# jspenmar/slowtv_monodepth

Hardware: AMD Instinct MI355X
Metric: training images/sec (640×192, 3-frame) at 1/2/4/8 MI355X; warp+SSIM HBM GB/s (higher is better)
Workload: dtype f32

## Files before the change

### include/smd_hotpath.h

```cpp
#ifndef SMD_HOTPATH_H
#define SMD_HOTPATH_H

#include <stddef.h>
#include <stdint.h>

#ifdef __cplusplus
extern "C" {
#endif

#define SMD_ABI_VERSION 8

#define SMD_OK 0
#define SMD_E_INVALID (-1)
#define SMD_E_LAUNCH (-2)
#define SMD_E_WORKSPACE (-3)
#define SMD_E_UNSUPPORTED (-4)

#define SMD_USE_MIN 0x1
#define SMD_USE_AUTOMASK 0x2
#define SMD_LOSS_L1 0x4
#define SMD_NEED_K_GRAD 0x8
#define SMD_USE_EDGES 0x10
#define SMD_LOSS_L2 0x20
#define SMD_MASK_EXPLAINABILITY 0x80
// ... 157 lines not shown
                                int B, int C, int CO, int h, int w, int pieces, void* stream);

size_t smd_conv3x3z_mfma_workspace_bytes(int B, int C, int CO, int h, int w);
int smd_conv3x3z_mfma_fwd(const float* x, const void* wp_fwd, float* y, void* workspace, size_t workspace_bytes,
                          int B, int C, int CO, int h, int w, int pieces, void* stream);
int smd_conv3x3z_mfma_bwd_data(const float* g_y, const void* wp_bwd, float* g_x, void* workspace, size_t workspace_bytes,
                               int B, int C, int CO, int h, int w, int pieces, void* stream);
int smd_conv3x3z_mfma_bwd_weight(const float* x, const float* g_y, float* g_weight, void* workspace, size_t workspace_bytes,
                                 int B, int C, int CO, int h, int w, int pieces, void* stream);

size_t smd_conv7x7s2_packed_bytes(int C, int CO);
size_t smd_conv7x7s2_workspace_bytes(int B, int C, int CO, int H, int W);
int smd_conv7x7s2_pack(const float* weight, void* wp, int C, int CO, void* stream);
int smd_conv7x7s2_fwd(const float* x, const void* wp, float* y, int B, int C, int CO, int H, int W, void* stream);
int smd_conv7x7s2_bwd_weight(const float* x, const float* g_y, float* g_weight, void* workspace, size_t workspace_bytes,
                             int B, int C, int CO, int H, int W, void* stream);

size_t smd_conv3x3s2_mfma_workspace_bytes(int B, int C, int CO, int H, int W);
int smd_conv3x3s2_mfma_fwd(const float* x, const void* wp_fwd, float* y, void* workspace, size_t workspace_bytes,
                           int B, int C, int CO, int H, int W, void* stream);
int smd_conv3x3s2_mfma_bwd_weight(const float* x, const float* g_y, float* g_weight, void* workspace, size_t workspace_bytes,
                                  int B, int C, int CO, int H, int W, void* stream);

size_t smd_bn_workspace_bytes(int N, int C, int HW);
int smd_bn_fwd(const float* x, const float* residual, const float* gamma, const float* beta, float* running_mean, float* running_var,
               float momentum, float eps, int relu, float* y, float* save_mean, float* save_invstd,
               void* workspace, size_t workspace_bytes, int N, int C, int HW, void* stream);
int smd_bn_bwd(const float* x, const float* y, const float* g_y, const float* gamma, const float* save_mean, const float* save_invstd,
               int relu, float* g_x, float* g_residual, float* g_gamma, float* g_beta,
               void* workspace, size_t workspace_bytes, int N, int C, int HW, void* stream);

int smd_maxpool3x3s2_fwd(const float* x, float* y, uint8_t* idx, int N, int C, int H, int W, void* stream);
int smd_maxpool3x3s2_bwd(const float* g_y, const uint8_t* idx, float* g_x, int N, int C, int H, int W, void* stream);

size_t smd_dwconv7x7_workspace_bytes(int C, int H, int W);
int smd_dwconv7x7_fwd(const float* x, const float* weight, const float* bias, float* y, int N, int C, int H, int W, int flip, void* stream);
int smd_dwconv7x7_wrw(const float* x, const float* g_y, float* g_weight, float* g_bias, void* workspace, size_t workspace_bytes,
                      int N, int C, int H, int W, void* stream);

size_t smd_layernorm_cf_workspace_bytes(int N, int C, int HW);
int smd_layernorm_cf_fwd(const float* x, const float* gamma, const float* beta, void* y, int y_is_bf16, float* mean, float* rstd,
                         int N, int C, int HW, float eps, void* stream);
int smd_layernorm_cf_bwd(const float* x, const void* g_y, int g_y_is_bf16, const float* gamma, const float* mean, const float* rstd,
                         float* g_x, float* g_gamma, float* g_beta, void* workspace, size_t workspace_bytes, int N, int C, int HW, void* stream);

size_t smd_channel_attention_workspace_bytes(int B, int C, int n, int backward);
// ... 114 lines not shown
```

### slowtv_monodepth_amd/_lib.py

```python
from __future__ import annotations

import ctypes as C
import os
from pathlib import Path

import torch

__all__ = ['lib', 'call', 'set_knob', 'reset_knobs', 'knob_epoch', 'lib_path', 'FLAGS', 'REGR_FLAGS', 'SEL_MASKED', 'ptr_array', 'int_array', 'i64_array', 'HotpathError', 'Unsupported']

_HERE = Path(__file__).resolve().parent
lib_path = Path(os.environ.get('SMD_HOTPATH_LIB', _HERE/'libsmd_hotpath.so'))

FLAGS = {'use_min': 0x1, 'use_automask': 0x2, 'loss_l1': 0x4, 'need_k_grad': 0x8, 'use_edges': 0x10, 'loss_l2': 0x20, 'packed_ready': 0x40,
         'mask_explainability': 0x80, 'mask_uncertainty': 0x100, 'use_laplacian': 0x200, 'bwd_skip_rows': 0x400, 'edges_ready': 0x800, 'bwd_no_live': 0x1000}
REGR_FLAGS = {'l1': 0x0, 'log_l1': 0x1, 'berhu': 0x2, 'invert': 0x4, 'automask': 0x8}
SEL_MASKED = 255
MAX_SCALES = 8
MAX_SUPPORTS = 8

_vp, _i, _f, _sz, _u64 = C.c_void_p, C.c_int, C.c_float, C.c_size_t, C.c_uint64

PROTOTYPES = {
    'smd_last_error': (C.c_char_p, []),
    'smd_abi_version': (_i, []),
# ... 50 lines not shown
    'smd_scale_mean_fwd': (_i, [_vp]*2 + [_i]*2 + [_vp]*2 + [_sz, _vp]),
    'smd_scale_mean_bwd': (_i, [_vp]*2 + [_i]*2 + [_vp]*3),
    'smd_conv3x3_thin_workspace_bytes': (_sz, [_i]*4),
    'smd_conv3x3_thin_fwd': (_i, [_vp]*3 + [_i]*4 + [_vp]),
    'smd_conv3x3_thin_bwd': (_i, [_vp]*6 + [_sz] + [_i]*4 + [_vp]),
    'smd_conv3x3_mfma_packed_bytes': (_sz, [_i]*3),
    'smd_conv3x3_mfma_workspace_bytes': (_sz, [_i]*5),
    'smd_conv3x3_mfma_pack': (_i, [_vp]*3 + [_i]*3 + [_vp]),
    'smd_conv3x3_mfma_fwd': (_i, [_vp]*4 + [_sz] + [_i]*6 + [_vp]),
    'smd_conv3x3_mfma_bwd_data': (_i, [_vp]*4 + [_sz] + [_i]*6 + [_vp]),
    'smd_conv3x3_mfma_bwd_weight': (_i, [_vp]*4 + [_sz] + [_i]*6 + [_vp]),
    'smd_conv3x3z_mfma_workspace_bytes': (_sz, [_i]*5),
    'smd_conv3x3z_mfma_fwd': (_i, [_vp]*4 + [_sz] + [_i]*6 + [_vp]),
    'smd_conv3x3z_mfma_bwd_data': (_i, [_vp]*4 + [_sz] + [_i]*6 + [_vp]),
    'smd_conv3x3z_mfma_bwd_weight': (_i, [_vp]*4 + [_sz] + [_i]*6 + [_vp]),
    'smd_conv7x7s2_packed_bytes': (_sz, [_i]*2),
    'smd_conv7x7s2_workspace_bytes': (_sz, [_i]*5),
    'smd_conv7x7s2_pack': (_i, [_vp]*2 + [_i]*2 + [_vp]),
    'smd_conv7x7s2_fwd': (_i, [_vp]*3 + [_i]*5 + [_vp]),
    'smd_conv7x7s2_bwd_weight': (_i, [_vp]*4 + [_sz] + [_i]*5 + [_vp]),
    'smd_conv3x3s2_mfma_workspace_bytes': (_sz, [_i]*5),
    'smd_conv3x3s2_mfma_fwd': (_i, [_vp]*4 + [_sz] + [_i]*5 + [_vp]),
    'smd_conv3x3s2_mfma_bwd_weight': (_i, [_vp]*4 + [_sz] + [_i]*5 + [_vp]),
    'smd_conv3x3_head_workspace_bytes': (_sz, [_i]*4),
    'smd_conv3x3_head_fwd': (_i, [_vp]*4 + [_i]*5 + [_vp]),
    'smd_conv3x3_head_bwd': (_i, [_vp]*8 + [_sz] + [_i]*5 + [_vp]),
    'smd_elu_pad_fwd': (_i, [_vp]*3 + [_i]*6 + [_vp]),
    'smd_elu_pad_bwd': (_i, [_vp]*6 + [_sz] + [_i]*6 + [_vp]),
    'smd_elu_up_cat_pad_fwd': (_i, [_vp]*4 + [_i]*6 + [_vp]),
    'smd_elu_up_cat_pad_bwd': (_i, [_vp]*7 + [_sz] + [_i]*6 + [_vp]),
    'smd_bn_workspace_bytes': (_sz, [_i, _i, _i]),
    'smd_bn_fwd': (_i, [_vp]*6 + [_f, _f, _i] + [_vp]*4 + [_sz] + [_i]*3 + [_vp]),
    'smd_bn_bwd': (_i, [_vp]*6 + [_i] + [_vp]*5 + [_sz] + [_i]*3 + [_vp]),
    'smd_maxpool3x3s2_fwd': (_i, [_vp]*3 + [_i]*4 + [_vp]),
    'smd_maxpool3x3s2_bwd': (_i, [_vp]*3 + [_i]*4 + [_vp]),
    'smd_dwconv7x7_workspace_bytes': (_sz, [_i]*3),
    'smd_dwconv7x7_fwd': (_i, [_vp]*4 + [_i]*5 + [_vp]),
    'smd_dwconv7x7_wrw': (_i, [_vp]*5 + [_sz] + [_i]*4 + [_vp]),
    'smd_layernorm_cf_workspace_bytes': (_sz, [_i]*3),
    'smd_layernorm_cf_fwd': (_i, [_vp]*4 + [_i] + [_vp]*2 + [_i]*3 + [_f, _vp]),
    'smd_layernorm_cf_bwd': (_i, [_vp]*2 + [_i] + [_vp]*7 + [_sz] + [_i]*3 + [_vp]),
    'smd_channel_attention_workspace_bytes': (_sz, [_i]*4),
    'smd_channel_attention_fwd': (_i, [_vp]*4 + [_sz] + [_i]*3 + [_vp]),
    'smd_channel_attention_bwd': (_i, [_vp]*5 + [_sz] + [_i]*3 + [_vp]),
    'smd_se_gate_workspace_bytes': (_sz, [_i]*3),
    'smd_se_gate_fwd': (_i, [_vp]*8 + [_sz] + [_i]*3 + [_vp]),
# ... 95 lines not shown
```

### slowtv_monodepth_amd/conv_routing.py

```python
from __future__ import annotations

import torch

from ._lib import Unsupported

_MODE = 'auto'
_ROUTES: dict = {}
_AB_WARMUPS, _AB_ROUNDS, _AB_MARGIN = 2, 5, 0.97
_DECLINED = (Unsupported, ValueError)


def set_conv_route(mode: str = 'auto'):
    global _MODE
    if mode not in ('auto', 'mfma', 'miopen'): raise ValueError(mode)
    _MODE = mode
    _ROUTES.clear()


def conv_routes() -> dict:
    return dict(_ROUTES)


_COARSE_W_MAX, _COARSE_C_MIN = 80, 256
_Z_FWD_WGT = [dict(px_min=1000, ch_max=511), dict(px_min=2400)]
STATIC_RULES = {
    'padded': {'fwd': [dict(thin=True), dict(thin=False, px_min=20000, c_co_max=128*64), dict(thin=False, coarse=True, px_min=1000)],
               'data': [dict(thin=True), dict(thin=False, px_min=5000, c_max=256), dict(thin=False, coarse=True, px_min=1000)],
               'wgt': [dict(thin=False, px_min=20000, co_max=64), dict(thin=False, coarse=True, px_min=2400)]},
    'bf16': {'fwd': [dict(thin=True)], 'data': [dict(thin=True)], 'wgt': [dict(thin=True)]},
    'zpad': {'fwd': _Z_FWD_WGT, 'data': [dict(px_min=1000)], 'wgt': _Z_FWD_WGT},
    'stem': {'fwd': [dict(px_min=20000)], 'wgt': [dict(px_min=20000)]},
}
_FAMILY_OF_SUFFIX = {'': 'padded', 'bf16': 'bf16', 'z': 'zpad', 's': 'stem'}
_BOUNDS = {'px_min': lambda v, B, C, CO, h, w: B*h*w >= v,
           'c_max': lambda v, B, C, CO, h, w: C <= v,
           'co_max': lambda v, B, C, CO, h, w: CO <= v,
           'c_co_max': lambda v, B, C, CO, h, w: C*CO <= v,
           'ch_max': lambda v, B, C, CO, h, w: max(C, CO) <= v,
           'thin': lambda v, B, C, CO, h, w: (CO == 16) == v,
           'coarse': lambda v, B, C, CO, h, w: (w <= _COARSE_W_MAX and C >= _COARSE_C_MIN) == v}


STRIDED_RULES = {
    's2': {'fwd': [dict(px_min=5000)], 'wgt': []},
}


def static_rule(op, B, C, CO, h, w) -> bool:
    kind, _, suffix = op.partition('_')
    clauses = STATIC_RULES[_FAMILY_OF_SUFFIX[suffix]][kind] if suffix in _FAMILY_OF_SUFFIX else STRIDED_RULES[suffix][kind]
    return any(all(_BOUNDS[name](v, B, C, CO, h, w) for name, v in clause.items()) for clause in clauses)


_capturing = torch.cuda.is_current_stream_capturing


def _time_interleaved(run_mfma, run_ref, rounds):
    ev = [[torch.cuda.Event(enable_timing=True) for _ in range(3)] for _ in range(rounds)]
    for e in ev:
        e[0].record(); run_mfma(); e[1].record(); run_ref(); e[2].record()
    torch.cuda.synchronize()
    return [e[0].elapsed_time(e[1])*1e3 for e in ev], [e[1].elapsed_time(e[2])*1e3 for e in ev]


def _conv_route(op, B, C, CO, h, w, run_mfma, run_ref) -> bool:
    if _MODE != 'auto': return _MODE == 'mfma'
    key = (op, B, C, CO, h, w)
    r = _ROUTES.get(key)
    if r is None:
        if _capturing(): return static_rule(op, B, C, CO, h, w)
        for _ in range(_AB_WARMUPS): run_mfma(); run_ref()
        us_m, us_r = _time_interleaved(run_mfma, run_ref, _AB_ROUNDS)
        t_m, t_r = sorted(us_m)[_AB_ROUNDS//2], sorted(us_r)[_AB_ROUNDS//2]
        r = _ROUTES[key] = (t_m < _AB_MARGIN*t_r, t_m, t_r)
# ... 18 lines not shown
```

### slowtv_monodepth_amd/conv_s2.py

```python
from __future__ import annotations

import torch

from . import _lib
from ._device import _check, _on, _stream, _workspace, call
from .conv_ops import _mfma_pack
from .conv_routing import serve


class _Conv3x3s2(torch.autograd.Function):
    @staticmethod
    def forward(ctx, x, weight):
        x = _check('x', x)
        if x.ndim != 4: raise ValueError(f'expected (B,C,H,W), got {tuple(x.shape)}')
        B, C, H, W = x.shape
        if weight.ndim != 4 or tuple(weight.shape[1:]) != (C, 3, 3): raise ValueError(f'weight: expected (CO,{C},3,3), got {tuple(weight.shape)}')
        CO = weight.shape[0]
        weight = _check('weight', weight, (CO, C, 3, 3))
        ho, wo = (H - 1)//2 + 1, (W - 1)//2 + 1
        nws = _lib.lib.smd_conv3x3s2_mfma_workspace_bytes(B, C, CO, H, W)
        y = torch.empty((B, CO, ho, wo), device=x.device, dtype=torch.float32)

        def run_mfma():
            wf = _mfma_pack(weight, C, CO, 3, True, False)[0]
            ws, n = _workspace(x.device, nws, floor=256)
            call('smd_conv3x3s2_mfma_fwd', x.data_ptr(), wf.data_ptr(), y.data_ptr(), ws.data_ptr(), n, B, C, CO, H, W, _stream())
            return y
        y = serve(('fwd_s2', B, C, CO, H, W), run_mfma, lambda: torch.conv2d(x, weight, None, 2, 1), eligible=nws > 0)
        ctx.save_for_backward(x, weight)
        ctx.nws = nws
        return y

    @staticmethod
    def backward(ctx, g_y):
        x, weight = ctx.saved_tensors
        dev = _on(x)
        B, C, H, W = x.shape
        CO = weight.shape[0]
        need_x, need_w = ctx.needs_input_grad
        g_y = _check('grad(y)', g_y, (B, CO, (H - 1)//2 + 1, (W - 1)//2 + 1))
        cb = lambda mask: torch.ops.aten.convolution_backward(g_y, x, weight, None, [2, 2], [1, 1], [1, 1], False, [0, 0], 1, mask)
        g_x = cb([True, False, False])[0] if need_x else None
        g_w = None
        if need_w:
            g_w = torch.empty_like(weight)

            def run_wgt():
                ws, n = _workspace(dev, ctx.nws, floor=256)
                call('smd_conv3x3s2_mfma_bwd_weight', x.data_ptr(), g_y.data_ptr(), g_w.data_ptr(), ws.data_ptr(), n, B, C, CO, H, W, _stream())
                return g_w
            g_w = serve(('wgt_s2', B, C, CO, H, W), run_wgt, lambda: cb([False, True, False])[1], eligible=ctx.nws > 0)
        return g_x, g_w


def conv3x3_s2(x, weight):
    return _Conv3x3s2.apply(x, weight)
```

### slowtv_monodepth_amd/csrc/smd_api.hip

```cpp
#include <limits.h>
#include <math.h>
#include <stdarg.h>
#include <stdio.h>
#include <stdlib.h>
#include <string.h>
#include <algorithm>

#include "smd_kernels.h"
#include "smd_smooth_dev.h"

namespace {

thread_local char g_err[512] = "";

int fail(int code, const char* fmt, ...) {
  va_list ap;
  va_start(ap, fmt);
  vsnprintf(g_err, sizeof(g_err), fmt, ap);
  va_end(ap);
  return code;
}

int check_launch(hipError_t e, const char* what) {
  if (e != hipSuccess) return fail(SMD_E_LAUNCH, "%s: %s", what, hipGetErrorString(e));
// ... 871 lines not shown
  if (!g_y || (!g_xp && !g_weight) || (g_xp && !weight) || (g_weight && (!xp || !workspace))) return fail(SMD_E_INVALID, "null pointer");
  if (C != 16 && C != 32 && C >= 1) return fail(SMD_E_UNSUPPORTED, "the thin convolution serves 16 or 32 input channels, not %d", C);
  if (!thin_sizes_ok(B, C, h, w)) return fail(SMD_E_INVALID, "invalid sizes B=%d C=%d h=%d w=%d", B, C, h, w);
  if (g_weight && workspace_bytes < smd_conv3x3_thin_workspace_bytes(B, C, h, w)) return fail(SMD_E_WORKSPACE, "workspace too small");
  hipStream_t st = (hipStream_t)stream;
  if (g_xp) { if (int rc = check_launch(smd::launch_conv_thin_bwd_data(g_y, weight, g_xp, B, C, h, w, st), "conv3x3_thin_bwd (data)")) return rc; }
  if (g_weight) { if (int rc = check_launch(smd::launch_conv_thin_bwd_wgt(xp, g_y, g_weight, (float*)workspace, B, C, h, w, st), "conv3x3_thin_bwd (weights)")) return rc; }
  return SMD_OK;
}
int smd_conv3x3_thin_fwd(const float* xp, const float* weight, float* y, int B, int C, int h, int w, void* stream) {
  if (!xp || !weight || !y) return fail(SMD_E_INVALID, "null pointer");
  if (C != 16 && C != 32 && C >= 1) return fail(SMD_E_UNSUPPORTED, "the thin convolution serves 16 or 32 input channels, not %d", C);
  if (!thin_sizes_ok(B, C, h, w)) return fail(SMD_E_INVALID, "invalid sizes B=%d C=%d h=%d w=%d", B, C, h, w);
  return check_launch(smd::launch_conv_thin_fwd(xp, weight, y, B, C, h, w, (hipStream_t)stream), "conv3x3_thin_fwd");
}
static bool mfma_sizes_ok(int B, int C, int CO, int h, int w) {
  return B >= 1 && C >= 1 && CO >= 1 && C <= 4096 && CO <= 4096 && h >= 1 && w >= 1 && h < 32768 && w < 32768 && (long long)(h + 2)*(w + 2) < (1ll << 30) &&
         (long long)B*((C + 31)/32)*((CO + 31)/32) < 65536 && (long long)C*(h + 2)*(w + 2) < (1ll << 29) && (long long)CO*h*w < (1ll << 29);
}
using smd::ConvOp;
static bool conv_two_tiles() { return knob("conv_two_tiles", 0) != 0; }
size_t smd_conv3x3_mfma_packed_bytes(int C, int CO, int pieces) {
  if (C < 1 || CO < 1 || pieces < 1 || pieces > 3) return 0;
  return align256(smd::conv_mfma_packed_elems(C, CO, pieces)*2);
}
static size_t mfma_workspace_bytes(bool zpad, int B, int C, int CO, int h, int w, bool two_tiles) {
  if (!mfma_sizes_ok(B, C, CO, h, w)) return 0;
  size_t n = std::max({(size_t)64, smd::conv_mfma_split_elems(ConvOp::Fwd, zpad, B, C, CO, h, w, two_tiles), smd::conv_mfma_split_elems(ConvOp::Data, zpad, B, C, CO, h, w, two_tiles)});
  if (smd::conv_mfma_served(ConvOp::Wgt, zpad, C, CO)) n = std::max(n, smd::conv_mfma_wgrad_partials(zpad, B, C, CO, h, w));
  return align256(n*sizeof(float));
}
size_t smd_conv3x3_mfma_workspace_bytes(int B, int C, int CO, int h, int w) { return mfma_workspace_bytes(false, B, C, CO, h, w, conv_two_tiles()); }
size_t smd_conv3x3z_mfma_workspace_bytes(int B, int C, int CO, int h, int w) { return mfma_workspace_bytes(true, B, C, CO, h, w, conv_two_tiles()); }
static int mfma_unserved(ConvOp op, bool zpad, int C, int CO) {
  const char* name[] = {"forward", "data gradient", "weight gradient"};
  return fail(SMD_E_UNSUPPORTED, "the %s%s does not serve C=%d CO=%d", zpad ? "zero-padded " : "", name[(int)op], C, CO);
}
static int mfma_check(ConvOp op, bool zpad, size_t workspace_bytes, int B, int C, int CO, int h, int w, int pieces, bool two_tiles) {
  if (zpad && pieces != 2 && pieces != 3) return fail(SMD_E_UNSUPPORTED, "the zero-padded forms take float tensors: pieces 2 or 3, not %d", pieces);
  if (pieces < 1 || pieces > 3) return fail(SMD_E_UNSUPPORTED, "pieces must be 1 (bfloat16 tensors), 2 or 3 (float tensors), not %d", pieces);
  if (!mfma_sizes_ok(B, C, CO, h, w)) return fail(SMD_E_INVALID, "invalid sizes B=%d C=%d CO=%d h=%d w=%d", B, C, CO, h, w);
  if (!smd::conv_mfma_served(op, zpad, C, CO)) return mfma_unserved(op, zpad, C, CO);
  if (workspace_bytes < mfma_workspace_bytes(zpad, B, C, CO, h, w, two_tiles)) return fail(SMD_E_WORKSPACE, "workspace too small");
  return SMD_OK;
}
int smd_conv3x3_mfma_pack(const float* weight, void* wp_fwd, void* wp_bwd, int C, int CO, int pieces, void* stream) {
  if (!weight || (!wp_fwd && !wp_bwd)) return fail(SMD_E_INVALID, "null pointer");
  if (pieces < 1 || pieces > 3) return fail(SMD_E_UNSUPPORTED, "pieces must be 1 (bfloat16 tensors), 2 or 3 (float tensors), not %d", pieces);
  if (C < 1 || CO < 1 || C > 4096 || CO > 4096) return fail(SMD_E_INVALID, "invalid sizes C=%d CO=%d", C, CO);
  if (wp_fwd && !smd::conv_mfma_served(ConvOp::Fwd, false, C, CO)) return mfma_unserved(ConvOp::Fwd, false, C, CO);
  if (wp_bwd && !smd::conv_mfma_served(ConvOp::Data, false, C, CO)) return mfma_unserved(ConvOp::Data, false, C, CO);
  return check_launch(smd::launch_conv_mfma_pack(weight, wp_fwd, wp_bwd, C, CO, pieces, (hipStream_t)stream), "conv3x3_mfma_pack");
}
static int mfma_form(ConvOp op, bool zpad, const void* in, const void* wp, void* out, void* workspace, size_t workspace_bytes, int B, int C, int CO, int h, int w, int pieces, void* stream, const char* what) {
  if (!in || !wp || !out || !workspace) return fail(SMD_E_INVALID, "null pointer");
  const bool two_tiles = conv_two_tiles();
  if (int rc = mfma_check(op, zpad, workspace_bytes, B, C, CO, h, w, pieces, two_tiles)) return rc;
  const auto launch = op == ConvOp::Fwd ? smd::launch_conv_mfma_fwd : smd::launch_conv_mfma_bwd_data;
  return check_launch(launch(in, wp, out, (float*)workspace, zpad, B, C, CO, h, w, pieces, two_tiles, (hipStream_t)stream), what);
}
static int mfma_bwd_weight(bool zpad, const void* x, const void* g_y, float* g_weight, void* workspace, size_t workspace_bytes, int B, int C, int CO, int h, int w, int pieces, void* stream) {
  if (!x || !g_y || !g_weight || !workspace) return fail(SMD_E_INVALID, "null pointer");
  if (int rc = mfma_check(ConvOp::Wgt, zpad, workspace_bytes, B, C, CO, h, w, pieces, conv_two_tiles())) return rc;
  return check_launch(smd::launch_conv_mfma_bwd_wgt(x, g_y, g_weight, (float*)workspace, zpad, B, C, CO, h, w, pieces, (hipStream_t)stream), zpad ? "conv3x3z_mfma_bwd_weight" : "conv3x3_mfma_bwd_weight");
}
int smd_conv3x3_mfma_fwd(const void* xp, const void* wp_fwd, void* y, void* workspace, size_t workspace_bytes, int B, int C, int CO, int h, int w, int pieces, void* stream) {
  return mfma_form(ConvOp::Fwd, false, xp, wp_fwd, y, workspace, workspace_bytes, B, C, CO, h, w, pieces, stream, "conv3x3_mfma_fwd");
}
int smd_conv3x3_mfma_bwd_data(const void* g_y, const void* wp_bwd, void* g_xp, void* workspace, size_t workspace_bytes, int B, int C, int CO, int h, int w, int pieces, void* stream) {
  return mfma_form(ConvOp::Data, false, g_y, wp_bwd, g_xp, workspace, workspace_bytes, B, C, CO, h, w, pieces, stream, "conv3x3_mfma_bwd_data");
}
int smd_conv3x3_mfma_bwd_weight(const void* xp, const void* g_y, float* g_weight, void* workspace, size_t workspace_bytes, int B, int C, int CO, int h, int w, int pieces, void* stream) {
  return mfma_bwd_weight(false, xp, g_y, g_weight, workspace, workspace_bytes, B, C, CO, h, w, pieces, stream);
}
// ... 39 lines not shown
  if (B < 1 || B > 65535 || C < 1 || CO < 1 || C > 4096 || CO > 4096 || H < 1 || W < 1) return false;
  const long long ho = (H - 1)/2 + 1, wo = (W - 1)/2 + 1;
  return (long long)C*H*W < (1ll << 29) && (long long)CO*ho*wo < (1ll << 29) && ho <= 65535 && (long long)B*((C + 63)/64)*((CO + 63)/64) < 65536;
}
size_t smd_conv3x3s2_mfma_workspace_bytes(int B, int C, int CO, int H, int W) {
  if (!smd::conv_s2_served(C, CO) || !s2_sizes_ok(B, C, CO, H, W)) return 0;
  return align256(smd::conv_s2_workspace_floats(B, C, CO, H, W)*sizeof(float));
}
static int s2_check(size_t workspace_bytes, int B, int C, int CO, int H, int W) {
  if (!smd::conv_s2_served(C, CO)) return fail(SMD_E_UNSUPPORTED, "the stride-2 kernels serve C %% 16 == 0 with CO %% 32 == 0, not C=%d CO=%d", C, CO);
  if (!s2_sizes_ok(B, C, CO, H, W)) return fail(SMD_E_UNSUPPORTED, "the stride-2 kernels do not serve B=%d C=%d CO=%d H=%d W=%d", B, C, CO, H, W);
  if (workspace_bytes < smd_conv3x3s2_mfma_workspace_bytes(B, C, CO, H, W)) return fail(SMD_E_WORKSPACE, "workspace too small");
  return SMD_OK;
}
int smd_conv3x3s2_mfma_fwd(const float* x, const void* wp_fwd, float* y, void* workspace, size_t workspace_bytes, int B, int C, int CO, int H, int W, void* stream) {
  if (!x || !wp_fwd || !y || !workspace) return fail(SMD_E_INVALID, "null pointer");
  if (int rc = s2_check(workspace_bytes, B, C, CO, H, W)) return rc;
  return check_launch(smd::launch_conv_s2_fwd(x, wp_fwd, y, (float*)workspace, B, C, CO, H, W, (hipStream_t)stream), "conv3x3s2_mfma_fwd");
}
int smd_conv3x3s2_mfma_bwd_weight(const float* x, const float* g_y, float* g_weight, void* workspace, size_t workspace_bytes, int B, int C, int CO, int H, int W, void* stream) {
  if (!x || !g_y || !g_weight || !workspace) return fail(SMD_E_INVALID, "null pointer");
  if (int rc = s2_check(workspace_bytes, B, C, CO, H, W)) return rc;
  return check_launch(smd::launch_conv_s2_bwd_wgt(x, g_y, g_weight, (float*)workspace, B, C, CO, H, W, (hipStream_t)stream), "conv3x3s2_mfma_bwd_weight");
}
int smd_elu_up_cat_pad_fwd(const void* a, const float* bias, const void* skip, void* out, int B, int Ca, int Cs, int h, int w, int dtypes, void* stream) {
  if (!a || !out || (Cs > 0 && !skip)) return fail(SMD_E_INVALID, "null pointer");
  if (B < 1 || Ca < 1 || Cs < 0 || h < 1 || w < 1 || !dec_sizes_ok((long long)B*(Ca + Cs), 2*h, 2*w))
    return fail(SMD_E_INVALID, "invalid sizes B=%d Ca=%d Cs=%d h=%d w=%d", B, Ca, Cs, h, w);
  return check_launch(smd::launch_elu_up_cat_pad_fwd(a, bias, skip, out, B, Ca, Cs, h, w, dtypes, (hipStream_t)stream), "elu_up_cat_pad_fwd");
}
int smd_elu_up_cat_pad_bwd(const void* a, const float* bias, const void* g_out, void* g_a, void* g_skip, float* g_bias,
                           void* workspace, size_t workspace_bytes, int B, int Ca, int Cs, int h, int w, int dtypes, void* stream) {
  if (!a || !g_out || (!g_a && !g_skip) || (g_bias && (!workspace || !g_a))) return fail(SMD_E_INVALID, "null pointer");
  if (B < 1 || Ca < 1 || Cs < 0 || h < 1 || w < 1 || !dec_sizes_ok((long long)B*(Ca + Cs), 2*h, 2*w))
    return fail(SMD_E_INVALID, "invalid sizes B=%d Ca=%d Cs=%d h=%d w=%d", B, Ca, Cs, h, w);
  if (g_bias && workspace_bytes < smd_decoder_glue_workspace_bytes(B, Ca, h, w)) return fail(SMD_E_WORKSPACE, "workspace too small");
  return check_launch(smd::launch_elu_up_cat_pad_bwd(a, bias, g_out, g_a, g_skip, g_bias, (float*)workspace, B, Ca, Cs, h, w, dtypes, (hipStream_t)stream),
                      "elu_up_cat_pad_bwd");
}

size_t smd_bn_workspace_bytes(int N, int C, int HW) {
  if (N < 1 || C < 1 || HW < 1) return 0;
  return align256(((size_t)C*smd::bn_chunks(N, HW)*3 + (size_t)C*3)*sizeof(float));
}
int smd_bn_fwd(const float* x, const float* residual, const float* gamma, const float* beta, float* running_mean, float* running_var,
               float momentum, float eps, int relu, float* y, float* save_mean, float* save_invstd, void* workspace, size_t workspace_bytes,
// ... 438 lines not shown
```

### slowtv_monodepth_amd/csrc/smd_conv_s2.hip

```cpp
#include "smd_common.h"
#include "smd_kernels.h"
#include "smd_conv_mfma_dev.h"
#include <algorithm>
#include <type_traits>

namespace smd {

namespace {

constexpr int kS2Pix = 388;

template <int P>
__global__ __launch_bounds__(256, 2) void k_conv_s2_fwd(const float* __restrict__ x, const uint4* __restrict__ wp, float* __restrict__ out,
                                                        int CK, int M, int H, int W, int ho, int wo, int TR, int TCW, int KS, int kc_per_split,
                                                        size_t split_stride, unsigned gx, unsigned gy, unsigned gz) {
  constexpr int NPIX = kS2Pix, kBuf = P*NPIX*2;
  __shared__ uint4 tile[2*kBuf];
  const int lane = threadIdx.x & 63, wall = __builtin_amdgcn_readfirstlane(threadIdx.x >> 6), j = lane & 31, g = lane >> 5;
  const int MT = M >> 5, MG = (MT + 3) >> 2;
  const unsigned nblk = (unsigned)(MG*KS)*gx*gy*gz, lid = xcd_block_id(nblk);
  if (lid >= nblk) return;
  const int mg_own = (int)(lid % MG)*4 + wall, mg = min(mg_own, MT - 1), ks = (lid/MG) % KS;
  const unsigned tl = lid/(MG*KS);
  const int x0 = (int)(tl % gx)*TCW, y0 = (int)((tl/gx) % gy)*TR, b = (int)(tl/(gx*gy));
// ... 258 lines not shown
#pragma unroll
      for (int r = 0; r < 16; ++r) {
        const int co = cog*T::COB + cot*32 + mfma32_row(r, g);
        if (co < CO) partial[((blk*9 + t)*CO + co)*C + c] = acc[t][r];
      }
  }
}

void s2_wgrad_shape(int B, int C, int CO, int ho, int wo, dim3& grid, int& rows, int& spb) {
  const int cgs = ceil_div(C, S2W::CB)*ceil_div(CO, S2W::COB), strips = ceil_div(wo, S2W::STRIP);
  const long long base = (long long)strips*B*cgs;
  const int groups = (int)std::max(1ll, std::min<long long>(256/std::max(base, 1ll), ceil_div(ho, 6)));
  rows = ceil_div(ho, groups);
  spb = 1;
  if (rows == ho && base > 512) spb = (int)std::min<long long>(B, base/256);
  grid = dim3(strips, ceil_div(ho, rows), ceil_div(B, spb)*cgs);
}
unsigned s2_wgrad_sets(int B, int C, int CO, int ho, int wo) {
  dim3 grid; int rows, spb;
  s2_wgrad_shape(B, C, CO, ho, wo, grid, rows, spb);
  return grid.x*grid.y*(unsigned)ceil_div(B, spb);
}

}

bool conv_s2_served(int C, int CO) { return C >= 16 && C % 16 == 0 && CO >= 32 && CO % 32 == 0; }
size_t conv_s2_workspace_floats(int B, int C, int CO, int H, int W) {
  const int ho = (H - 1)/2 + 1, wo = (W - 1)/2 + 1;
  const S2Shape s = s2_fwd_shape(B, C, CO, ho, wo);
  return std::max({(size_t)64, s.KS > 1 ? (size_t)s.KS*s.out_elems : (size_t)0, partial_sets_floats(s2_wgrad_sets(B, C, CO, ho, wo), (size_t)9*CO*C)});
}
hipError_t launch_conv_s2_fwd(const float* x, const void* wp_fwd, float* y, float* split_ws, int B, int C, int CO, int H, int W, hipStream_t st) {
  const int ho = (H - 1)/2 + 1, wo = (W - 1)/2 + 1;
  const S2Shape s = s2_fwd_shape(B, C, CO, ho, wo);
  hipLaunchKernelGGL(k_conv_s2_fwd<3>, s.grid, dim3(256), 0, st, x, (const uint4*)wp_fwd, s.KS > 1 ? split_ws : y, C, CO, H, W, ho, wo, s.TR, s.TCW, s.KS, s.kcs,
                     s.out_elems, s.gx, s.gy, s.gz);
  if (s.KS > 1) {
    const size_t n4 = s.out_elems/4;
    hipLaunchKernelGGL(k_s2_split_sum, dim3((unsigned)((n4 + 255)/256)), dim3(256), 0, st, split_ws, y, n4, s.KS);
  }
  return hipGetLastError();
}
hipError_t launch_conv_s2_bwd_wgt(const float* x, const float* gy, float* g_w, float* partial, int B, int C, int CO, int H, int W, hipStream_t st) {
  const int ho = (H - 1)/2 + 1, wo = (W - 1)/2 + 1;
  dim3 grid; int rows, spb;
  s2_wgrad_shape(B, C, CO, ho, wo, grid, rows, spb);
  hipLaunchKernelGGL(k_conv_s2_wgrad, grid, dim3(256), 0, st, x, gy, partial, B, C, CO, H, W, ho, wo, rows, spb);
  return launch_partial_sets_finalize(partial, grid.x*grid.y*(unsigned)ceil_div(B, spb), 9*CO*C, SetIndexMap{CO, C}, g_w, st);
}

}
```

### slowtv_monodepth_amd/csrc/smd_kernels.h

```cpp
#pragma once
#include <hip/hip_runtime.h>
#include <stddef.h>
#include <stdint.h>

#include "../../include/smd_hotpath.h"

namespace smd {

constexpr int kFwdCols = 62;
constexpr int kBwdCols = 60;
#ifndef SMD_WAVES_PER_BLOCK
#define SMD_WAVES_PER_BLOCK 4
#endif
constexpr int kWavesPerBlock = SMD_WAVES_PER_BLOCK;
#ifndef SMD_SMOOTH_CHUNK
#define SMD_SMOOTH_CHUNK 1024
#endif
constexpr int kSmoothChunk = SMD_SMOOTH_CHUNK;
__host__ __device__ inline int smooth_chunk_px(int n) { return n > 32768 ? kSmoothChunk : 256; }
__host__ __device__ inline int smooth_chunks_of(int n) { return (n + smooth_chunk_px(n) - 1)/smooth_chunk_px(n); }
constexpr int kSmoothCols = 63, kSmoothRows = 8;
__host__ __device__ inline int smooth_units_of(int hs, int ws) { return ((ws + kSmoothCols - 1)/kSmoothCols)*((hs + kSmoothRows - 1)/kSmoothRows); }
constexpr int kSmoothRowsMain = 16;
__host__ __device__ inline int smooth_units_main(int hs, int ws) { return ((ws + kSmoothCols - 1)/kSmoothCols)*((hs + kSmoothRowsMain - 1)/kSmoothRowsMain); }
// ... 214 lines not shown
  if (op == ConvOp::Data) return (CO % 16 == 0 && C % 32 == 0) || (thin && C == 16);
  return CO % 32 == 0 || thin;
}
size_t conv_mfma_packed_elems(int C, int CO, int pieces);
size_t conv_mfma_wgrad_partials(bool zpad, int B, int C, int CO, int h, int w);
size_t conv_mfma_split_elems(ConvOp op, bool zpad, int B, int C, int CO, int h, int w, bool two_tiles);
hipError_t launch_conv_mfma_pack(const float* w, void* wp_fwd, void* wp_bwd, int C, int CO, int pieces, hipStream_t st);
hipError_t launch_conv_mfma_fwd(const void* x, const void* wp_fwd, void* y, float* split_ws, bool zpad, int B, int C, int CO, int h, int w, int pieces, bool two_tiles, hipStream_t st);
hipError_t launch_conv_mfma_bwd_data(const void* gy, const void* wp_bwd, void* g_x, float* split_ws, bool zpad, int B, int C, int CO, int h, int w, int pieces, bool two_tiles, hipStream_t st);
hipError_t launch_conv_mfma_bwd_wgt(const void* x, const void* gy, float* g_w, float* partial, bool zpad, int B, int C, int CO, int h, int w, int pieces, hipStream_t st);
struct SetIndexMap { int CO = 0, C = 0; };
size_t partial_sets_floats(unsigned T, size_t n);
hipError_t launch_partial_sets_finalize(float* partial, unsigned T, int n, SetIndexMap index_map, float* g_w, hipStream_t st);
bool conv_stem_served(int C, int CO);
size_t conv_stem_packed_bytes(int C);
size_t conv_stem_wgrad_floats(int B, int C, int H, int W);
hipError_t launch_conv_stem_pack(const float* w, void* wp, int C, hipStream_t st);
hipError_t launch_conv_stem_fwd(const float* x, const void* wp, float* y, int B, int C, int H, int W, hipStream_t st);
hipError_t launch_conv_stem_bwd_wgt(const float* x, const float* gy, float* g_w, float* partial, int B, int C, int H, int W, hipStream_t st);
bool conv_s2_served(int C, int CO);
size_t conv_s2_workspace_floats(int B, int C, int CO, int H, int W);
hipError_t launch_conv_s2_fwd(const float* x, const void* wp_fwd, float* y, float* split_ws, int B, int C, int CO, int H, int W, hipStream_t st);
hipError_t launch_conv_s2_bwd_wgt(const float* x, const float* gy, float* g_w, float* partial, int B, int C, int CO, int H, int W, hipStream_t st);
size_t decoder_bias_partials(int B, int C, int h, int w);
hipError_t launch_elu_pad_fwd(const void* x, const float* bias, void* out, int B, int C, int h, int w, int apply_elu, int dt, hipStream_t st);
hipError_t launch_elu_pad_bwd(const void* x, const float* bias, const void* g_out, void* g_x, float* g_bias, float* ws, int B, int C, int h, int w,
                              int apply_elu, int dt, hipStream_t st);
hipError_t launch_elu_up_cat_pad_fwd(const void* a, const float* bias, const void* skip, void* out, int B, int Ca, int Cs, int h, int w, int dt,
                                     hipStream_t st);
hipError_t launch_elu_up_cat_pad_bwd(const void* a, const float* bias, const void* g_out, void* g_a, void* g_skip, float* g_bias, float* ws,
                                     int B, int Ca, int Cs, int h, int w, int dt, hipStream_t st);
hipError_t launch_relu_pad_fwd(const float* x, const float* bias, float* out, int B, int C, int h, int w, hipStream_t st);
hipError_t launch_relu_pad_bwd(const float* x, const float* bias, const float* g_out, float* g_x, float* g_bias, float* ws, int B, int C, int h, int w,
                               hipStream_t st);
struct UpCatGate { int B, Ca, Cs, h, w, R, act; };
bool up_cat_gate_sizes_ok(const UpCatGate& s);
size_t up_cat_gate_workspace_floats(const UpCatGate& s);
hipError_t launch_up_cat_gate_pad_fwd(const UpCatGate& s, const float* a, const float* bias, const float* skip, const float* w1, const float* w2, float* out,
                                      float* gate, float* mean, float* hid, float* ws, hipStream_t st);
hipError_t launch_up_cat_gate_pad_bwd(const UpCatGate& s, const float* a, const float* bias, const float* skip, const float* w1, const float* w2,
                                      const float* gate, const float* mean, const float* hid, const float* g_out, float* g_a, float* g_skip, float* g_bias,
                                      float* g_w1, float* g_w2, float* ws, hipStream_t st);
struct SubPixel { int B, C, Cs, h, w, r, pre_act, act, pad; };
bool subpixel_sizes_ok(const SubPixel& s);
size_t subpixel_workspace_floats(const SubPixel& s);
hipError_t launch_subpixel_fwd(const SubPixel& s, const float* x, const float* pre_bias, const float* weight, const float* bias, const float* skip, float* out,
// ... 147 lines not shown
```

Before: 952.5.

## Add MFMA backward-data kernel for stride-2 3x3 convolutions with routing

Measured after the change: 962.5 (median of 6 runs). 1.01x the previous value.

```diff
diff --git a/include/smd_hotpath.h b/include/smd_hotpath.h
--- a/include/smd_hotpath.h
+++ b/include/smd_hotpath.h
@@ -203,6 +203,10 @@
 int smd_conv3x3s2_mfma_bwd_weight(const float* x, const float* g_y, float* g_weight, void* workspace, size_t workspace_bytes,
                                   int B, int C, int CO, int H, int W, void* stream);
 
+size_t smd_conv3x3s2d_mfma_workspace_bytes(int B, int C, int CO, int H, int W);
+int smd_conv3x3s2d_mfma_bwd_data(const float* g_y, const void* wp_bwd, float* g_x, void* workspace, size_t workspace_bytes,
+                                 int B, int C, int CO, int H, int W, void* stream);
+
 size_t smd_bn_workspace_bytes(int N, int C, int HW);
 int smd_bn_fwd(const float* x, const float* residual, const float* gamma, const float* beta, float* running_mean, float* running_var,
                float momentum, float eps, int relu, float* y, float* save_mean, float* save_invstd,
diff --git a/slowtv_monodepth_amd/_lib.py b/slowtv_monodepth_amd/_lib.py
--- a/slowtv_monodepth_amd/_lib.py
+++ b/slowtv_monodepth_amd/_lib.py
@@ -96,6 +96,8 @@
     'smd_conv3x3s2_mfma_workspace_bytes': (_sz, [_i]*5),
     'smd_conv3x3s2_mfma_fwd': (_i, [_vp]*4 + [_sz] + [_i]*5 + [_vp]),
     'smd_conv3x3s2_mfma_bwd_weight': (_i, [_vp]*4 + [_sz] + [_i]*5 + [_vp]),
+    'smd_conv3x3s2d_mfma_workspace_bytes': (_sz, [_i]*5),
+    'smd_conv3x3s2d_mfma_bwd_data': (_i, [_vp]*4 + [_sz] + [_i]*5 + [_vp]),
     'smd_conv3x3_head_workspace_bytes': (_sz, [_i]*4),
     'smd_conv3x3_head_fwd': (_i, [_vp]*4 + [_i]*5 + [_vp]),
     'smd_conv3x3_head_bwd': (_i, [_vp]*8 + [_sz] + [_i]*5 + [_vp]),
diff --git a/slowtv_monodepth_amd/conv_routing.py b/slowtv_monodepth_amd/conv_routing.py
--- a/slowtv_monodepth_amd/conv_routing.py
+++ b/slowtv_monodepth_amd/conv_routing.py
@@ -46,10 +46,24 @@
 }
 
 
+TRANSPOSED_RULES = {
+    't2': {'data': [dict(px_min=5000)]},
+}
+
+
 def static_rule(op, B, C, CO, h, w) -> bool:
     kind, _, suffix = op.partition('_')
-    clauses = STATIC_RULES[_FAMILY_OF_SUFFIX[suffix]][kind] if suffix in _FAMILY_OF_SUFFIX else STRIDED_RULES[suffix][kind]
+    if suffix in _FAMILY_OF_SUFFIX: clauses = STATIC_RULES[_FAMILY_OF_SUFFIX[suffix]][kind]
+    elif suffix in STRIDED_RULES or suffix not in TRANSPOSED_RULES: clauses = STRIDED_RULES[suffix][kind]
+    else: clauses = TRANSPOSED_RULES[suffix][kind]
     return any(all(_BOUNDS[name](v, B, C, CO, h, w) for name, v in clause.items()) for clause in clauses)
+
+
+def may_serve(key, unknown=True) -> bool:
+    if _MODE != 'auto': return _MODE == 'mfma'
+    r = _ROUTES.get(key)
+    if r is None: return static_rule(*key) if torch.cuda.is_initialized() and _capturing() else unknown
+    return r[0]
 
 
 _capturing = torch.cuda.is_current_stream_capturing
diff --git a/slowtv_monodepth_amd/conv_s2.py b/slowtv_monodepth_amd/conv_s2.py
--- a/slowtv_monodepth_amd/conv_s2.py
+++ b/slowtv_monodepth_amd/conv_s2.py
@@ -5,7 +5,7 @@
 from . import _lib
 from ._device import _check, _on, _stream, _workspace, call
 from .conv_ops import _mfma_pack
-from .conv_routing import serve
+from .conv_routing import may_serve, serve
 
 
 class _Conv3x3s2(torch.autograd.Function):
@@ -19,29 +19,41 @@
         weight = _check('weight', weight, (CO, C, 3, 3))
         ho, wo = (H - 1)//2 + 1, (W - 1)//2 + 1
         nws = _lib.lib.smd_conv3x3s2_mfma_workspace_bytes(B, C, CO, H, W)
+        nwd = _lib.lib.smd_conv3x3s2d_mfma_workspace_bytes(B, C, CO, H, W) if ctx.needs_input_grad[0] else 0
+        want_bwd = nwd > 0 and may_serve(('data_t2', B, C, CO, H, W)) and may_serve(('fwd_s2', B, C, CO, H, W), unknown=False)
         y = torch.empty((B, CO, ho, wo), device=x.device, dtype=torch.float32)
+        packed = {}
 
         def run_mfma():
-            wf = _mfma_pack(weight, C, CO, 3, True, False)[0]
+            wf, packed['wb'] = _mfma_pack(weight, C, CO, 3, True, want_bwd)
             ws, n = _workspace(x.device, nws, floor=256)
             call('smd_conv3x3s2_mfma_fwd', x.data_ptr(), wf.data_ptr(), y.data_ptr(), ws.data_ptr(), n, B, C, CO, H, W, _stream())
             return y
         y = serve(('fwd_s2', B, C, CO, H, W), run_mfma, lambda: torch.conv2d(x, weight, None, 2, 1), eligible=nws > 0)
-        ctx.save_for_backward(x, weight)
-        ctx.nws = nws
+        ctx.save_for_backward(x, weight, packed.get('wb'))
+        ctx.nws, ctx.nwd = nws, nwd
         return y
 
     @staticmethod
     def backward(ctx, g_y):
-        x, weight = ctx.saved_tensors
+        x, weight, wp_bwd = ctx.saved_tensors
         dev = _on(x)
         B, C, H, W = x.shape
         CO = weight.shape[0]
         need_x, need_w = ctx.needs_input_grad
         g_y = _check('grad(y)', g_y, (B, CO, (H - 1)//2 + 1, (W - 1)//2 + 1))
         cb = lambda mask: torch.ops.aten.convolution_backward(g_y, x, weight, None, [2, 2], [1, 1], [1, 1], False, [0, 0], 1, mask)
-        g_x = cb([True, False, False])[0] if need_x else None
-        g_w = None
+        g_x = g_w = None
+        if need_x:
+            g_x = torch.empty_like(x)
+            packed = {'wb': wp_bwd}
+
+            def run_data():
+                if packed['wb'] is None: packed['wb'] = _mfma_pack(weight, C, CO, 3, False, True)[1]
+                ws, n = _workspace(dev, ctx.nwd, floor=256)
+                call('smd_conv3x3s2d_mfma_bwd_data', g_y.data_ptr(), packed['wb'].data_ptr(), g_x.data_ptr(), ws.data_ptr(), n, B, C, CO, H, W, _stream())
+                return g_x
+            g_x = serve(('data_t2', B, C, CO, H, W), run_data, lambda: cb([True, False, False])[0], eligible=ctx.nwd > 0)
         if need_w:
             g_w = torch.empty_like(weight)
 
diff --git a/slowtv_monodepth_amd/csrc/smd_api.hip b/slowtv_monodepth_amd/csrc/smd_api.hip
--- a/slowtv_monodepth_amd/csrc/smd_api.hip
+++ b/slowtv_monodepth_amd/csrc/smd_api.hip
@@ -917,7 +917,7 @@
 static bool conv_two_tiles() { return knob("conv_two_tiles", 0) != 0; }
 size_t smd_conv3x3_mfma_packed_bytes(int C, int CO, int pieces) {
   if (C < 1 || CO < 1 || pieces < 1 || pieces > 3) return 0;
-  return align256(smd::conv_mfma_packed_elems(C, CO, pieces)*2);
+  return align256(smd::conv_mfma_packed_elems((C + 31) & ~31, CO, pieces)*2);
 }
 static size_t mfma_workspace_bytes(bool zpad, int B, int C, int CO, int h, int w, bool two_tiles) {
   if (!mfma_sizes_ok(B, C, CO, h, w)) return 0;
@@ -944,7 +944,7 @@
   if (pieces < 1 || pieces > 3) return fail(SMD_E_UNSUPPORTED, "pieces must be 1 (bfloat16 tensors), 2 or 3 (float tensors), not %d", pieces);
   if (C < 1 || CO < 1 || C > 4096 || CO > 4096) return fail(SMD_E_INVALID, "invalid sizes C=%d CO=%d", C, CO);
   if (wp_fwd && !smd::conv_mfma_served(ConvOp::Fwd, false, C, CO)) return mfma_unserved(ConvOp::Fwd, false, C, CO);
-  if (wp_bwd && !smd::conv_mfma_served(ConvOp::Data, false, C, CO)) return mfma_unserved(ConvOp::Data, false, C, CO);
+  if (wp_bwd && !smd::conv_mfma_served(ConvOp::Data, false, C, CO) && !(pieces == 3 && smd::conv_s2_served(C, CO))) return mfma_unserved(ConvOp::Data, false, C, CO);
   return check_launch(smd::launch_conv_mfma_pack(weight, wp_fwd, wp_bwd, C, CO, pieces, (hipStream_t)stream), "conv3x3_mfma_pack");
 }
 static int mfma_form(ConvOp op, bool zpad, const void* in, const void* wp, void* out, void* workspace, size_t workspace_bytes, int B, int C, int CO, int h, int w, int pieces, void* stream, const char* what) {
@@ -1030,6 +1030,18 @@
   if (!x || !g_y || !g_weight || !workspace) return fail(SMD_E_INVALID, "null pointer");
   if (int rc = s2_check(workspace_bytes, B, C, CO, H, W)) return rc;
   return check_launch(smd::launch_conv_s2_bwd_wgt(x, g_y, g_weight, (float*)workspace, B, C, CO, H, W, (hipStream_t)stream), "conv3x3s2_mfma_bwd_weight");
+}
+static bool s2d_sizes_ok(int B, int C, int CO, int H, int W) { return s2_sizes_ok(B, C, CO, H, W) && smd::conv_s2d_blocks(B, C, CO, H, W) < (1ll << 31); }
+size_t smd_conv3x3s2d_mfma_workspace_bytes(int B, int C, int CO, int H, int W) {
+  if (!smd::conv_s2_served(C, CO) || !s2d_sizes_ok(B, C, CO, H, W)) return 0;
+  return align256(smd::conv_s2d_workspace_floats(B, C, CO, H, W)*sizeof(float));
+}
+int smd_conv3x3s2d_mfma_bwd_data(const float* g_y, const void* wp_bwd, float* g_x, void* workspace, size_t workspace_bytes, int B, int C, int CO, int H, int W, void* stream) {
+  if (!g_y || !wp_bwd || !g_x || !workspace) return fail(SMD_E_INVALID, "null pointer");
+  if (!smd::conv_s2_served(C, CO)) return fail(SMD_E_UNSUPPORTED, "the stride-2 kernels serve C %% 16 == 0 with CO %% 32 == 0, not C=%d CO=%d", C, CO);
+  if (!s2d_sizes_ok(B, C, CO, H, W)) return fail(SMD_E_UNSUPPORTED, "the stride-2 kernels do not serve B=%d C=%d CO=%d H=%d W=%d", B, C, CO, H, W);
+  if (workspace_bytes < smd_conv3x3s2d_mfma_workspace_bytes(B, C, CO, H, W)) return fail(SMD_E_WORKSPACE, "workspace too small");
+  return check_launch(smd::launch_conv_s2_bwd_data(g_y, wp_bwd, g_x, (float*)workspace, B, C, CO, H, W, (hipStream_t)stream), "conv3x3s2d_mfma_bwd_data");
 }
 int smd_elu_up_cat_pad_fwd(const void* a, const float* bias, const void* skip, void* out, int B, int Ca, int Cs, int h, int w, int dtypes, void* stream) {
   if (!a || !out || (Cs > 0 && !skip)) return fail(SMD_E_INVALID, "null pointer");
diff --git a/slowtv_monodepth_amd/csrc/smd_conv_s2.hip b/slowtv_monodepth_amd/csrc/smd_conv_s2.hip
--- a/slowtv_monodepth_amd/csrc/smd_conv_s2.hip
+++ b/slowtv_monodepth_amd/csrc/smd_conv_s2.hip
@@ -304,6 +304,161 @@
   return grid.x*grid.y*(unsigned)ceil_div(B, spb);
 }
 
+constexpr int kS2DPix = 128;
+
+__device__ __forceinline__ constexpr int s2d_slot(int s) { return (int)((0x867250134ull >> (4*s)) & 15); }
+
+template <int P>
+__device__ __forceinline__ void split_mfma_two(const bf16x8 (&A0)[P], const bf16x8 (&B0)[P], f32x16& acc0, f32x16& lo0,
+                                               const bf16x8 (&A1)[P], const bf16x8 (&B1)[P], f32x16& acc1, f32x16& lo1) {
+  constexpr int NPROD = n_products(P);
+#pragma unroll
+  for (int t = 0; t < NPROD; ++t) {
+    if (t == NPROD - 1) { acc0 = mfma_bf16(A0[0], B0[0], acc0); acc1 = mfma_bf16(A1[0], B1[0], acc1); }
+    else {
+      lo0 = mfma_bf16(A0[prod_a(P, t)], B0[prod_b(P, t)], lo0);
+      lo1 = mfma_bf16(A1[prod_a(P, t)], B1[prod_b(P, t)], lo1);
+    }
+  }
+}
+
+template <int P>
+__global__ __launch_bounds__(256, 2) void k_conv_s2_bwd_data(const float* __restrict__ gy, const uint4* __restrict__ wp, float* __restrict__ out,
+                                                             int CK, int M, int H, int W, int ho, int wo, int TR, int TCW, int KS, int kc_per_split,
+                                                             size_t split_stride, unsigned gx, unsigned gyb, unsigned gz) {
+  constexpr int NPIX = kS2DPix, kBuf = P*NPIX*2;
+  __shared__ uint4 tile[2*kBuf];
+  const int lane = threadIdx.x & 63, wall = __builtin_amdgcn_readfirstlane(threadIdx.x >> 6), j = lane & 31, g = lane >> 5;
+  const int MT = (M + 31) >> 5, MG = (MT + 1) >> 1;
+  const unsigned nblk = (unsigned)(MG*KS)*gx*gyb*gz, lid = xcd_block_id(nblk);
+  if (lid >= nblk) return;
+  const int nf = wall & 1;
+  const int mt_own = (int)(lid % MG)*2 + (wall >> 1), mt = min(mt_own, MT - 1), ks = (lid/MG) % KS;
+  const unsigned tl = lid/(MG*KS);
+  const int c0 = (int)(tl % gx)*TCW, r0 = (int)((tl/gx) % gyb)*TR, b = (int)(tl/(gx*gyb));
+  const int PW = TCW + 1, NP = (TR + 1)*PW;
+  const int KC = CK >> 4, kc0 = ks*kc_per_split, kc1 = min(KC, kc0 + kc_per_split);
+  const size_t plane = (size_t)ho*wo;
+  const float* src = gy + (size_t)b*CK*plane;
+
+  const int p = nf*32 + j, r = p/TCW, c = p - r*TCW;
+  const bool have = p < TR*TCW && r0 + r < ho && c0 + c < wo;
+  const int lbase = have ? r*PW + c : 0;
+
+  using Stage = PatchStager<256, NPIX, P, float, true>;
+  constexpr int TRIPS = Stage::TRIPS;
+  Stage stage;
+#pragma unroll
+  for (int t = 0; t < TRIPS; ++t) {
+    const int item = Stage::item(t), half = item >= NPIX ? 1 : 0, pix = item - half*NPIX;
+    const int rp = pix/PW, q = pix - rp*PW;
+    const int yy = r0 + rp, xx = c0 + q;
+    stage.pofs[t] = (pix < NP && yy < ho && xx < wo) ? yy*wo + xx : -1;
+  }
+  float v[TRIPS][8];
+  auto request = [&](int kc) { stage.request(src, plane, kc, v); };
+
+  f32x16 acc[4], lo[4];
+#pragma unroll
+  for (int q = 0; q < 4; ++q)
+#pragma unroll
+    for (int rr = 0; rr < 16; ++rr) { acc[q][rr] = 0.f; lo[q][rr] = 0.f; }
+
+  bf16x8 A[5][P], Bf[2][P];
+  const uint4* wq = wp + ((size_t)mt*KC*9*P)*64 + lane;
+  auto fetch_a = [&](bf16x8 (&dst)[P], int kc, int s) {
+#pragma unroll
+    for (int pc = 0; pc < P; ++pc) dst[pc] = as_frag(wq[(size_t)((kc*9 + s2d_slot(s))*P + pc)*64]);
+  };
+  auto read_b = [&](bf16x8 (&dst)[P], int buf, int d) { Stage::read(tile, buf, lbase + d, g, dst); };
+  auto chunk = [&](int kc, int cur, auto more_tag) {
+    constexpr bool MORE = decltype(more_tag)::value;
+    read_b(Bf[0], cur, 0);
+    read_b(Bf[1], cur, 1);
+    split_mfma_two<P>(A[0], Bf[0], acc[0], lo[0], A[1], Bf[0], acc[1], lo[1]);
+    fetch_a(A[4], kc, 4); fetch_a(A[0], kc, 5);
+    __builtin_amdgcn_sched_barrier(0);
+    split_mfma_two<P>(A[2], Bf[0], acc[2], lo[2], A[3], Bf[0], acc[3], lo[3]);
+    fetch_a(A[1], kc, 6); fetch_a(A[2], kc, 7);
+    read_b(Bf[0], cur, PW);
+    if (MORE) request(kc + 1);
+    __builtin_amdgcn_sched_barrier(0);
+    split_mfma_two<P>(A[4], Bf[1], acc[1], lo[1], A[0], Bf[1], acc[3], lo[3]);
+    fetch_a(A[3], kc, 8);
+    if (MORE) fetch_a(A[0], kc + 1, 0);
+    read_b(Bf[1], cur, PW + 1);
+    __builtin_amdgcn_sched_barrier(0);
+    split_mfma_two<P>(A[1], Bf[0], acc[2], lo[2], A[2], Bf[0], acc[3], lo[3]);
+    if (MORE) { fetch_a(A[1], kc + 1, 1); fetch_a(A[2], kc + 1, 2); }
+    __builtin_amdgcn_sched_barrier(0);
+    split_mfma<P>(A[3], Bf[1], acc[3], lo[3]);
+    if (MORE) {
+      fetch_a(A[3], kc + 1, 3);
+      stage.file(tile, cur ^ 1, v);
+    }
+    __builtin_amdgcn_sched_barrier(0);
+    __syncthreads();
+  };
+
+  if (kc0 < kc1) {
+    request(kc0);
+#pragma unroll
+    for (int s = 0; s < 4; ++s) fetch_a(A[s], kc0, s);
+    stage.file(tile, 0, v);
+  }
+  __syncthreads();
+  int kc = kc0;
+  for (; kc + 1 < kc1; ++kc) chunk(kc, (kc - kc0) & 1, std::true_type{});
+  if (kc < kc1) chunk(kc, (kc - kc0) & 1, std::false_type{});
+
+  if (mt_own >= MT || !have) return;
+  float* dst = out + (size_t)ks*split_stride;
+  const int y = 2*(r0 + r), x = 2*(c0 + c);
+  const bool row1 = y + 1 < H, col1 = x + 1 < W;
+  const bool pairs = (W & 1) == 0 && (reinterpret_cast<uintptr_t>(dst) & 7) == 0;
+#pragma unroll
+  for (int rr = 0; rr < 16; ++rr) {
+    const int m = mt*32 + mfma32_row(rr, g);
+    if (m >= M) continue;
+    float* q = dst + (((size_t)b*M + m)*H + y)*W + x;
+    const float v00 = acc[0][rr] + lo[0][rr], v01 = acc[1][rr] + lo[1][rr], v10 = acc[2][rr] + lo[2][rr], v11 = acc[3][rr] + lo[3][rr];
+    if (pairs) {
+      *reinterpret_cast<f32x2v*>(q) = f32x2v{v00, v01};
+      if (row1) *reinterpret_cast<f32x2v*>(q + W) = f32x2v{v10, v11};
+    } else {
+      q[0] = v00;
+      if (col1) q[1] = v01;
+      if (row1) { q[W] = v10; if (col1) q[W + 1] = v11; }
+    }
+  }
+}
+
+void s2d_tile(int ho, int wo, int& TR, int& TCW) {
+  double best = -1.0; int best_patch = 0;
+  TR = 1; TCW = 1;
+  for (int tcw = std::min(wo, 63); tcw >= 1; --tcw) {
+    int tr = std::min(64/tcw, ho);
+    while (tr > 1 && (tr + 1)*(tcw + 1) > kS2DPix) --tr;
+    const int patch = (tr + 1)*(tcw + 1);
+    const double useful = (double)ho*wo/((double)ceil_div(ho, tr)*ceil_div(wo, tcw)*64.0);
+    if (useful > best + 1e-9 || (useful > best - 1e-9 && patch < best_patch)) { best = useful; best_patch = patch; TR = tr; TCW = tcw; }
+  }
+}
+S2Shape s2d_shape(int B, int C, int CO, int H, int W) {
+  const int ho = (H - 1)/2 + 1, wo = (W - 1)/2 + 1;
+  S2Shape s;
+  s2d_tile(ho, wo, s.TR, s.TCW);
+  s.gx = ceil_div(wo, s.TCW); s.gy = ceil_div(ho, s.TR); s.gz = B;
+  const int KC = CO >> 4, MG = ceil_div(ceil_div(C, 32), 2);
+  const long long base = (long long)s.gx*s.gy*s.gz*MG;
+  int ks = 1;
+  if (base < 256) ks = (int)std::min<long long>(std::max(KC/2, 1), (512 + base - 1)/base);
+  s.kcs = ceil_div(KC, ks); s.KS = ceil_div(KC, s.kcs);
+  s.grid = dim3(8*(unsigned)ceil_div(base*s.KS, 8ll));
+  s.out_elems = (size_t)B*C*H*W;
+  return s;
+}
+
 }
 
 bool conv_s2_served(int C, int CO) { return C >= 16 && C % 16 == 0 && CO >= 32 && CO % 32 == 0; }
@@ -331,4 +486,21 @@
   return launch_partial_sets_finalize(partial, grid.x*grid.y*(unsigned)ceil_div(B, spb), 9*CO*C, SetIndexMap{CO, C}, g_w, st);
 }
 
-}
+long long conv_s2d_blocks(int B, int C, int CO, int H, int W) { return (long long)s2d_shape(B, C, CO, H, W).grid.x; }
+size_t conv_s2d_workspace_floats(int B, int C, int CO, int H, int W) {
+  const S2Shape s = s2d_shape(B, C, CO, H, W);
+  return std::max((size_t)64, s.KS > 1 ? (size_t)s.KS*s.out_elems : (size_t)0);
+}
+hipError_t launch_conv_s2_bwd_data(const float* gy, const void* wp_bwd, float* g_x, float* split_ws, int B, int C, int CO, int H, int W, hipStream_t st) {
+  const int ho = (H - 1)/2 + 1, wo = (W - 1)/2 + 1;
+  const S2Shape s = s2d_shape(B, C, CO, H, W);
+  hipLaunchKernelGGL(k_conv_s2_bwd_data<3>, s.grid, dim3(256), 0, st, gy, (const uint4*)wp_bwd, s.KS > 1 ? split_ws : g_x, CO, C, H, W, ho, wo, s.TR, s.TCW, s.KS,
+                     s.kcs, s.out_elems, s.gx, s.gy, s.gz);
+  if (s.KS > 1) {
+    const size_t n4 = s.out_elems/4;
+    hipLaunchKernelGGL(k_s2_split_sum, dim3((unsigned)((n4 + 255)/256)), dim3(256), 0, st, split_ws, g_x, n4, s.KS);
+  }
+  return hipGetLastError();
+}
+
+}
diff --git a/slowtv_monodepth_amd/csrc/smd_kernels.h b/slowtv_monodepth_amd/csrc/smd_kernels.h
--- a/slowtv_monodepth_amd/csrc/smd_kernels.h
+++ b/slowtv_monodepth_amd/csrc/smd_kernels.h
@@ -260,6 +260,9 @@
 size_t conv_s2_workspace_floats(int B, int C, int CO, int H, int W);
 hipError_t launch_conv_s2_fwd(const float* x, const void* wp_fwd, float* y, float* split_ws, int B, int C, int CO, int H, int W, hipStream_t st);
 hipError_t launch_conv_s2_bwd_wgt(const float* x, const float* gy, float* g_w, float* partial, int B, int C, int CO, int H, int W, hipStream_t st);
+long long conv_s2d_blocks(int B, int C, int CO, int H, int W);
+size_t conv_s2d_workspace_floats(int B, int C, int CO, int H, int W);
+hipError_t launch_conv_s2_bwd_data(const float* gy, const void* wp_bwd, float* g_x, float* split_ws, int B, int C, int CO, int H, int W, hipStream_t st);
 size_t decoder_bias_partials(int B, int C, int h, int w);
 hipError_t launch_elu_pad_fwd(const void* x, const float* bias, void* out, int B, int C, int h, int w, int apply_elu, int dt, hipStream_t st);
 hipError_t launch_elu_pad_bwd(const void* x, const float* bias, const void* g_out, void* g_x, float* g_bias, float* ws, int B, int C, int h, int w,
```
